# angelocatalani/neural-network-compression

Measured on AMD Instinct MI355X. Metric: weights/sec through prune+k-means (K=256), higher is better.
Workload: dtype f32

## Files before the change

### neural_network_compression_amd/csrc/nnc_hip.hip

```cpp
#include "nnc_common.hpp"
#include "nnc_km_shared.hpp"


extern "C" size_t nnc_kmeans_workspace_bytes(int32_t k)
{
    (void)k;
    return sizeof(KmWs) + 256;
}

extern "C" int32_t nnc_fix_shift(float absmax, int64_t n_total)
{
    int L = 1;
    while (((int64_t)1 << L) < n_total && L < 62) L++;
    if (!(absmax > 0.0f) || !std::isfinite(absmax)) return 0;
    int P = 0;
    (void)std::frexp((double)absmax, &P);
    return std::min(28, 62 - L) - P;
}

__device__ __forceinline__ int fix_f32(float v, int Sft)
{
    return (int)rintf(ldexpf(v, Sft));
}

// ... 3168 lines not shown
    unsigned char *b = reinterpret_cast<unsigned char *>(scratch_dev);
    float *cand_x = reinterpret_cast<float *>(b); b += reloc_align((size_t)cap * 4);
    float *cand_d = reinterpret_cast<float *>(b); b += reloc_align((size_t)cap * 4);
    KmWin *win = reinterpret_cast<KmWin *>(b); b += reloc_align(16 * (size_t)(p->k + 2));
    int *meta = reinterpret_cast<int *>(b); b += reloc_align(16);
    long long *keys = reinterpret_cast<long long *>(b); b += reloc_align(8 * (size_t)NNC_KMAX);
    unsigned *hist0 = reinterpret_cast<unsigned *>(b);
    int glog2, rlog2;
    km_defaults(p, &glog2, &rlog2);
    const size_t lds = km_lds_bytes(p->k, glog2, rlog2, false) + (NNC_KMAX + 2) * sizeof(int);
    if (lds > 128 * 1024) return fail(NNC_EINVAL, "relocation: search tables too large for the candidate kernel");
    if (!g_reloc_dist_attr[current_device()].load(std::memory_order_acquire)) {
        HIPCHK(hipFuncSetAttribute(reinterpret_cast<const void *>(&k_reloc_dist), hipFuncAttributeMaxDynamicSharedMemorySize, 128 * 1024));
        g_reloc_dist_attr[current_device()].store(1, std::memory_order_release);
    }
    NNC_LAUNCH_PROF(NNC_PROF_RELOC, k_reloc_head, dim3(KM_GMAX / KM_THREADS + 1), dim3(KM_THREADS), 0, S(stream), x_sorted, (long long)p->n, w, (long long)cap, win, meta,
                       hist0, (int)wmax);
    LAUNCHCHK("k_reloc_head");
    const int grid = (int)std::max<int64_t>(1, std::min<int64_t>(128, (2 * (int64_t)64 * (p->k + 1) + KM_THREADS - 1) / KM_THREADS));
    NNC_LAUNCH_PROF(NNC_PROF_RELOC, k_reloc_dist, dim3(grid), dim3(KM_THREADS), lds, S(stream), x_sorted, (const KmWin *)win, (const int *)meta, cand_x, cand_d, (long long)cap,
                       reinterpret_cast<const KmWs *>(w), hist0, 1);
    LAUNCHCHK("k_reloc_dist");
#ifndef KM_CHAIN_FIVE
    if (p->k > 256 && !km_fused(p) && p->prefix_dev) {
        unsigned char *hb = reinterpret_cast<unsigned char *>(host_mapped);
        NNC_LAUNCH_PROF(NNC_PROF_RELOC, k_reloc_select_finalize, dim3(1), dim3(KM_THREADS), 0, S(stream), w, (const float *)cand_x, (const float *)cand_d, (const KmWin *)win,
                        (const int *)meta, keys, (const unsigned *)hist0, reinterpret_cast<nnc_kmeans_status *>(hb),
                        reinterpret_cast<unsigned long long *>(hb ? hb + sizeof(nnc_kmeans_status) : nullptr), (unsigned long long)ticket, 1 | (p->k << 8));
        LAUNCHCHK("k_reloc_select_finalize");
        return NNC_OK;
    }
#endif
    NNC_LAUNCH_PROF(NNC_PROF_RELOC, k_reloc_select, dim3(1), dim3(KM_THREADS), 0, S(stream), w, (const float *)cand_x, (const float *)cand_d, (const KmWin *)win, (const int *)meta, 0, keys, 1, (const unsigned *)hist0, 1);
    LAUNCHCHK("k_reloc_select");
    return km_launch_finalize(w, p, FIN_FROM_PARTIALS, 2, stream, host_mapped, ticket);
}


int nnc_wait_ticket_(void *host_ticket, uint64_t ticket, void *stream)
{
    return km_wait_ticket(reinterpret_cast<volatile unsigned long long *>(host_ticket), (unsigned long long)ticket, S(stream));
}
int km_wait_ticket(volatile unsigned long long *word, unsigned long long ticket, hipStream_t stream)
{
    unsigned long long spins = 0;
    bool synced = false;
    auto t0 = std::chrono::steady_clock::now();
    while (__atomic_load_n(word, __ATOMIC_ACQUIRE) != ticket) {
        if ((++spins & 0x3FFF) == 0) {
            const double el = std::chrono::duration<double>(std::chrono::steady_clock::now() - t0).count();
            if (el > 0.02 && !synced) {
                hipError_t e = hipStreamSynchronize(stream);
                if (e != hipSuccess) return fail(NNC_EHIP, std::string("nnc_kmeans_fit: ") + hipGetErrorString(e));
                synced = true;
            } else if (el > 60.0) return fail(NNC_EHIP, "nnc_kmeans_fit: the status never arrived");
        }
    }
    return NNC_OK;
}

extern "C" int nnc_kmeans_fit(const float *x_iter, void *ws, const nnc_kmeans_params *pp, int32_t max_batch, int32_t sorted,
                              void *reloc_scratch_dev, size_t reloc_scratch_bytes, void *host_mapped, uint64_t *ticket_io,
                              nnc_kmeans_status *status_out, int32_t *n_windowed_out, void *stream)
{
    int rc = km_check(ws, pp, "nnc_kmeans_fit");
    if (rc) return rc;
    if (!host_mapped || !ticket_io || !status_out || (reinterpret_cast<uintptr_t>(host_mapped) & 7) != 0) return fail(NNC_EINVAL, "nnc_kmeans_fit: null / unaligned pointer");
    const nnc_kmeans_params p = *pp;
    if (p.n != p.n_total) return fail(NNC_EINVAL, "nnc_kmeans_fit: single GPU only (sharded fits: nnc_kmeans_iterate_sharded)");
    if (max_batch < 1) max_batch = 1;
    const bool lloyd = km_lloyd_ok(&p, x_iter);
    const bool one_launch = !lloyd && km_one_launch_fit(&p, x_iter);
    const size_t slot = sizeof(nnc_kmeans_status) + 8;
    unsigned char *hb = reinterpret_cast<unsigned char *>(host_mapped);
    const bool spec_ok = sorted && !one_launch && p.prefix_dev && reloc_scratch_dev && (reinterpret_cast<uintptr_t>(reloc_scratch_dev) & 255) == 0 &&
                         reloc_scratch_bytes >= nnc_kmeans_reloc_scratch_bytes(p.k, KM_SPEC_WMAX) && p.n >= 2 * KM_SPEC_WMAX;
    const bool mass_in_place = (p.flags & NNC_KM_MASS_IN_PLACE) && !lloyd && p.k > 64;
    bool spec = spec_ok && !mass_in_place;
    int batch = one_launch ? p.max_iter : (spec_ok ? 6 : 1);
    if (lloyd) batch = KM_LLOYD_ROUNDS;
    bool first_launch = true;
    int nwin = 0, nrel_seen = status_out->n_relocated, nunp_seen = status_out->n_unproven;
    int nip_seen = status_out->n_in_place;
    if (!spec_ok) { nrel_seen = 0; nunp_seen = 0; nip_seen = 0; }
    double s_prev = -1.0, s_last = -1.0;
    int i_prev = 0, i_last = 0;
    KmWs *w = reinterpret_cast<KmWs *>(ws);
    for (;;) {
        const uint64_t ticket = ++(*ticket_io);
        unsigned char *sl = hb + (ticket & 1) * slot;
        if (lloyd) {
            if ((rc = km_set_lds_attr())) return rc;
            for (int i = 0; i < batch; i++) {
                const bool last = i == batch - 1;
                if ((rc = km_launch_lloyd_round(x_iter, w, &p, first_launch ? p.max_iter : -1, stream, (last && !spec) ? sl : nullptr, ticket, spec ? 1 : 0))) return rc;
                first_launch = false;
                if (spec && (rc = km_launch_spec_reloc(x_iter, w, &p, reloc_scratch_dev, stream, last ? sl : nullptr, ticket))) return rc;
            }
        } else if (spec) {
            if ((rc = km_set_lds_attr())) return rc;
            for (int i = 0; i < batch; i++) {
                if ((rc = km_launch_accumulate(x_iter, w, &p, stream))) return rc;
                if ((rc = km_launch_finalize(w, &p, FIN_FROM_SHARDS, 0, stream, nullptr, 0, false, x_iter))) return rc;
                if ((rc = km_launch_spec_reloc(x_iter, w, &p, reloc_scratch_dev, stream, i == batch - 1 ? sl : nullptr, ticket))) return rc;
            }
        } else {
            const int lag = (!one_launch && batch >= 4) ? KM_FIT_LAG : 0;
            if ((rc = km_iterate_publish_(x_iter, ws, &p, batch, sl, ticket, stream, spec_ok, lag))) return rc;
        }
        if ((rc = km_wait_ticket(reinterpret_cast<volatile unsigned long long *>(sl + sizeof(nnc_kmeans_status)), ticket, S(stream)))) return rc;
        const nnc_kmeans_status st = *reinterpret_cast<const nnc_kmeans_status *>(sl);
        *status_out = st;
        const int dev_events = spec_ok ? st.n_relocated - nrel_seen : 0;
        const int chain_events = dev_events - (spec_ok ? st.n_in_place - nip_seen : 0);
        nrel_seen = st.n_relocated;
        nip_seen = st.n_in_place;
        nwin += dev_events;
        nwin += spec_ok ? st.n_unproven - nunp_seen : 0;
        nunp_seen = st.n_unproven;
        if (st.done) break;
        if (lloyd && !st.paused) continue;
        if (spec && !st.paused) {
            if (2 * chain_events >= batch) { batch = 4; s_prev = s_last = -1.0; continue; }
            spec = false;
            s_prev = s_last = -1.0;
        }
        if (st.paused) {
            const bool strict_check = st.iter >= 1 && st.same_counts;
            const int32_t window = (sorted && st.paused == 1 && !strict_check) ? nnc_kmeans_reloc_window(p.n, st.n_empty) : 0;
            if (window == 0 || !reloc_scratch_dev || reloc_scratch_bytes < nnc_kmeans_reloc_scratch_bytes(p.k, window)) break;
            if ((rc = nnc_kmeans_relocate_windowed(x_iter, ws, &p, st.n_empty, reloc_scratch_dev, reloc_scratch_bytes, stream))) return rc;
            nwin++;
            if (!lloyd) batch = one_launch ? p.max_iter : 1;
            s_prev = s_last = -1.0;
            continue;
        }
        if (one_launch) continue;
        s_prev = s_last; i_prev = i_last;
        s_last = (double)st.shift_tot; i_last = st.iter;
        batch = std::min(max_batch, batch * 2);
        if (s_prev > 0.0 && s_last > 0.0 && s_prev > s_last && p.tol > 0.0f) {
            const double rate = std::log(s_prev / s_last) / std::max(1, i_last - i_prev);
            const double left = s_last > (double)p.tol ? std::log(s_last / (double)p.tol) / rate : 0.0;
            batch = (int)std::max(1.0, std::min((double)max_batch, std::floor(left * 0.9)));
        }
    }
    if (n_windowed_out) *n_windowed_out = nwin;
    return NNC_OK;
}

extern "C" int nnc_kmeans_reloc_select_local(const float *x_sorted, void *ws, const nnc_kmeans_params *p, int32_t n_empty,
                                             void *scratch_dev, size_t scratch_bytes, int64_t *keys_out_dev, void *stream)
{
    int rc = km_check(ws, p, "nnc_kmeans_reloc_select_local");
    if (rc) return rc;
    const int32_t window = nnc_kmeans_reloc_window(p->n, n_empty);
    if (window == 0) return fail(NNC_EINVAL, "nnc_kmeans_reloc_select_local: not applicable (nnc_kmeans_reloc_window() == 0)");
    if (!x_sorted || !scratch_dev || !keys_out_dev || (reinterpret_cast<uintptr_t>(scratch_dev) & 255) != 0)
        return fail(NNC_EINVAL, "nnc_kmeans_reloc_select_local: null or unaligned (256 B) pointer");
    if (scratch_bytes < nnc_kmeans_reloc_scratch_bytes(p->k, window)) return fail(NNC_ENOSPACE, "nnc_kmeans_reloc_select_local: scratch too small");
    const int64_t cap = reloc_cap(p->k, window);
    unsigned char *b = reinterpret_cast<unsigned char *>(scratch_dev);
    float *cand_x = reinterpret_cast<float *>(b); b += reloc_align((size_t)cap * 4);
    float *cand_d = reinterpret_cast<float *>(b); b += reloc_align((size_t)cap * 4);
    void *win = b; b += reloc_align(16 * (size_t)(p->k + 2));
    int32_t *meta = reinterpret_cast<int32_t *>(b); b += reloc_align(16) + reloc_align(8 * (size_t)NNC_KMAX);
    unsigned *hist0 = reinterpret_cast<unsigned *>(b);
    if ((rc = km_reloc_windows_dist(x_sorted, ws, p, window, cand_x, cand_d, cap, win, meta, hist0, stream))) return rc;
    NNC_LAUNCH_PROF(NNC_PROF_RELOC, k_reloc_select, dim3(1), dim3(KM_THREADS), 0, S(stream), reinterpret_cast<KmWs *>(ws), cand_x, cand_d,
                       reinterpret_cast<const KmWin *>(win), reinterpret_cast<const int *>(meta), (int)n_empty,
                       reinterpret_cast<long long *>(keys_out_dev), 0, (const unsigned *)hist0, 0);
    LAUNCHCHK("k_reloc_select");
    return NNC_OK;
}

extern "C" int32_t *nnc_kmeans_reloc_flag(void *ws)
{
    if (!ws) return nullptr;
    return &reinterpret_cast<KmWs *>(ws)->reloc_fail;
}

__global__ __launch_bounds__(KM_THREADS) void k_relocate_if_proven(KmWs *__restrict__ ws, const long long *__restrict__ keys, int nkeys)
{
    __shared__ KmRelocLds lds;
    if (ws->reloc_fail) return;
    km_relocate_body(ws, keys, nkeys, &lds);
}

extern "C" int nnc_kmeans_relocate_if_proven(void *ws, const int64_t *keys_sorted_dev, int32_t nkeys, void *stream)
{
    if (!ws || !keys_sorted_dev || nkeys < 1) return fail(NNC_EINVAL, "nnc_kmeans_relocate_if_proven: bad argument");
    hipLaunchKernelGGL(k_relocate_if_proven, dim3(1), dim3(KM_THREADS), 0, S(stream), reinterpret_cast<KmWs *>(ws),
                       reinterpret_cast<const long long *>(keys_sorted_dev), nkeys);
    LAUNCHCHK("k_relocate_if_proven");
    return NNC_OK;
}

template <typename LT>
__global__ __launch_bounds__(256) void k_labels_equal(const LT *__restrict__ a, const LT *__restrict__ b, int64_t n, int *flag)
{
    const int64_t tid = (int64_t)blockIdx.x * blockDim.x + threadIdx.x;
    const int64_t nthreads = (int64_t)gridDim.x * blockDim.x;
    int diff = 0;
    for (int64_t i = tid; i < n; i += nthreads) diff |= (a[i] != b[i]);
    if (__any(diff) && (threadIdx.x & 63) == 0) *flag = 0;
}
__global__ void k_set_i32(int *p, int v) { *p = v; }
__global__ void k_set_done_if(KmWs *ws, const int *flag, int code) { if (*flag) ws->st.done = code; }

extern "C" int nnc_labels_equal(const void *a, const void *b, int64_t n, int label_bytes, int32_t *flag_dev, void *stream)
{
    if (!flag_dev || n < 0 || (n > 0 && (!a || !b))) return fail(NNC_EINVAL, "nnc_labels_equal: bad argument");
    hipLaunchKernelGGL(k_set_i32, dim3(1), dim3(1), 0, S(stream), flag_dev, 1);
    LAUNCHCHK("k_set_i32");
    if (n == 0) return NNC_OK;
    const int64_t bytes = n * label_bytes;
    if (((reinterpret_cast<uintptr_t>(a) | reinterpret_cast<uintptr_t>(b)) & 7) == 0 && (bytes & 7) == 0) {
        int grid = stream_grid(bytes / 8, 256 * 4, 8);
        hipLaunchKernelGGL((k_labels_equal<unsigned long long>), dim3(grid), dim3(256), 0, S(stream), reinterpret_cast<const unsigned long long *>(a), reinterpret_cast<const unsigned long long *>(b), bytes / 8, flag_dev);
    } else if (label_bytes == 1) {
        int grid = stream_grid(n, 256 * 4, 8);
        hipLaunchKernelGGL((k_labels_equal<uint8_t>), dim3(grid), dim3(256), 0, S(stream), reinterpret_cast<const uint8_t *>(a), reinterpret_cast<const uint8_t *>(b), n, flag_dev);
    } else {
        int grid = stream_grid(n, 256 * 4, 8);
        hipLaunchKernelGGL((k_labels_equal<uint16_t>), dim3(grid), dim3(256), 0, S(stream), reinterpret_cast<const uint16_t *>(a), reinterpret_cast<const uint16_t *>(b), n, flag_dev);
    }
    LAUNCHCHK("k_labels_equal");
// ... 64 lines not shown
```

### neural_network_compression_amd/csrc/nnc_layer.hip

```cpp
#include <hip/hip_runtime.h>

#include <algorithm>
#include <cmath>
#include <cstdint>
#include <cstring>
#include <string>
#include <vector>

#include "nnc.h"

int nnc_set_error_(int code, const char *msg);
int nnc_publish_bytes_(const void *src_dev, void *dst_host_mapped, int nbytes, void *host_ticket, uint64_t ticket, void *stream);
int nnc_wait_ticket_(void *host_ticket, uint64_t ticket, void *stream);
int nnc_sort_pruned_bounded_flagged_(const float *x, int64_t n, int64_t n_neg, int64_t n_zero, float vmin, float vmax, float thr,
                                     float *sorted_out, void *ws, size_t ws_bytes, int32_t *flag_dev, void *stream);

extern "C" int nnc_host_linspace_f32(float start, float stop, int32_t num, float *out)
{
    if (num < 0 || (num > 0 && !out)) return nnc_set_error_(NNC_EINVAL, "nnc_host_linspace_f32: bad argument");
    if (num == 0) return NNC_OK;
    const int div = num - 1;
    const volatile float delta = stop - start;
    if (div > 0) {
        const volatile float step = delta / (float)div;
        for (int i = 0; i < num; i++) {
            volatile float y = (float)i;
            if (step == 0.0f) { y = y / (float)div; y = y * delta; }
            else y = y * step;
            y = y + start;
            out[i] = y;
        }
        out[num - 1] = stop;
    } else {
        volatile float y = 0.0f;
        y = y * delta;
        y = y + start;
        out[0] = y;
    }
    return NNC_OK;
}

static void linspace_f64(double start, double stop, int num, double *out)
{
    const int div = num - 1;
    const volatile double delta = stop - start;
    if (div > 0) {
        const volatile double step = delta / (double)div;
        for (int i = 0; i < num; i++) {
            volatile double y = (double)i;
            if (step == 0.0) { y = y / (double)div; y = y * delta; }
            else y = y * step;
            y = y + start;
            out[i] = y;
        }
        out[num - 1] = stop;
    } else if (num == 1) {
        volatile double y = 0.0;
        y = y * delta;
        out[0] = y + start;
    }
}

extern "C" int nnc_host_cdf(const float *steps32, const int64_t *counts31, float *xnew300, double *cdf300)
{
    if (!steps32 || !counts31 || !xnew300 || !cdf300) return nnc_set_error_(NNC_EINVAL, "nnc_host_cdf: null pointer");
    const float *x = steps32;
    int64_t tot = 0;
    for (int i = 0; i < 31; i++) tot += counts31[i];
    double cdf[31];
    volatile double acc = 0.0;
    for (int i = 0; i < 31; i++) {
        const volatile double t = (double)counts31[i] / (double)tot;
        acc = (i == 0) ? (double)t : acc + t;
        cdf[i] = acc;
    }
    const double last = cdf[30];
    for (int i = 0; i < 31; i++) { const volatile double q = cdf[i] / last; cdf[i] = q; }
    float xmin = x[0], xmax = x[0];
    for (int i = 1; i < 31; i++) { xmin = std::min(xmin, x[i]); xmax = std::max(xmax, x[i]); }
    int rc = nnc_host_linspace_f32(xmin, xmax, 300, xnew300);
    if (rc) return rc;
    for (int j = 0; j < 300; j++) {
        const float v = xnew300[j];
        int idx = (int)(std::lower_bound(x, x + 31, v) - x);
        idx = std::min(std::max(idx, 1), 30);
        const int lo = idx - 1, hi = idx;
        const volatile float dx = x[hi] - x[lo];
        const volatile double dy = cdf[hi] - cdf[lo];
        const volatile double slope = dy / (double)dx;
        const volatile float xr = v - x[lo];
        const volatile double prod = slope * (double)xr;
        cdf300[j] = prod + cdf[lo];
    }
    return NNC_OK;
}

extern "C" int nnc_host_density_init(const float *xnew300, const double *cdf300, int32_t bits, float *space_out)
{
    if (!xnew300 || !cdf300 || !space_out || bits < 0 || bits > 10) return nnc_set_error_(NNC_EINVAL, "nnc_host_density_init: bad argument");
    const int k = (1 << bits) + 1;
    std::vector<double> tmp((size_t)k);
    linspace_f64(0.0, 1.0, k, tmp.data());
    for (int t = 0; t < k; t++) {
        int best = 0;
        double bd = std::fabs(cdf300[0] - tmp[t]);
        for (int j = 1; j < 300; j++) {
            const double d = std::fabs(cdf300[j] - tmp[t]);
            if (d < bd) { bd = d; best = j; }
        }
        space_out[t] = xnew300[best];
    }
    return NNC_OK;
}

static size_t al(size_t b) { return (b + 255) & ~(size_t)255; }

struct SideStream { int dev = -1; hipStream_t stream = nullptr; hipEvent_t fork = nullptr, join = nullptr; };
static int side_stream(SideStream **out)
{
    static thread_local SideStream side;
    int dev = 0;
    if (hipGetDevice(&dev) != hipSuccess) return nnc_set_error_(NNC_EHIP, "hipGetDevice failed");
    if (side.dev != dev) {
        if (side.stream) { (void)hipStreamDestroy(side.stream); (void)hipEventDestroy(side.fork); (void)hipEventDestroy(side.join); side = SideStream(); }
        if (hipStreamCreateWithFlags(&side.stream, hipStreamNonBlocking) != hipSuccess || hipEventCreateWithFlags(&side.fork, hipEventDisableTiming) != hipSuccess ||
            hipEventCreateWithFlags(&side.join, hipEventDisableTiming) != hipSuccess)
            return nnc_set_error_(NNC_EHIP, "could not create the second stream");
        side.dev = dev;
    }
    *out = &side;
    return NNC_OK;
}

struct LayerLayout {
    size_t prune_ws, stats_out, stats_ws, sorted, sort_ws, km_ws, prefix, reloc, back, small_out, total;
    size_t prune_ws_bytes, stats_ws_bytes, sort_ws_bytes, km_ws_bytes, prefix_bytes, reloc_bytes;
};

static LayerLayout layer_layout(int64_t n, int32_t k)
{
    LayerLayout L;
    size_t o = 0;
    auto take = [&](size_t bytes) { const size_t at = o; o += al(bytes); return at; };
    L.prune_ws_bytes = nnc_prune_stats_workspace_bytes(n);
    L.stats_ws_bytes = std::max(nnc_layer_stats_workspace_bytes(n), nnc_minmax_workspace_bytes(n));
    L.sort_ws_bytes = std::max(std::max(nnc_sort_workspace_bytes(n), nnc_sort_pruned_workspace_bytes(n, 0, (n + 3) / 4)),
                               nnc_sort_pruned_bounded_workspace_bytes(n - (n + 3) / 4));
    L.km_ws_bytes = nnc_kmeans_workspace_bytes(k);
    L.prefix_bytes = nnc_kmeans_prefix_bytes(n);
    L.reloc_bytes = n >= 512 ? nnc_kmeans_reloc_scratch_bytes(k, 256) : 0;
    L.prune_ws = take(std::max<size_t>(L.prune_ws_bytes, 16));
    L.stats_out = take(512);
    L.stats_ws = take(std::max<size_t>(L.stats_ws_bytes, 16));
    L.sorted = take((size_t)n * 4 + 16);
    L.sort_ws = take(std::max<size_t>(L.sort_ws_bytes, 16));
    L.km_ws = take(L.km_ws_bytes);
    L.prefix = take(std::max<size_t>(L.prefix_bytes, 16));
    L.reloc = take(std::max<size_t>(L.reloc_bytes, 16));
    L.back = take((size_t)k * 12);
    L.small_out = take(64 + 256);
    L.total = o + 256;
    return L;
}

extern "C" size_t nnc_compress_layer_workspace_bytes(int64_t n, int32_t k)
{
    if (n < 1 || k < 1 || k > NNC_KMAX - 8) return 0;
    return layer_layout(n, k).total;
}

extern "C" size_t nnc_compress_layer_host_bytes(void) { return 24576; }

#define LCHK(call) do { int rc_ = (call); if (rc_) return rc_; } while (0)
#define LHIP(call) do { hipError_t e_ = (call); if (e_ != hipSuccess) return nnc_set_error_(NNC_EHIP, hipGetErrorString(e_)); } while (0)

extern "C" int nnc_compress_layer_f32(float *x, int64_t n, const nnc_layer_params *lp, uint8_t *mask_out, void *labels_out,
                                      float *values_out, void *ws_dev, size_t ws_bytes, void *host_pinned, size_t host_bytes,
                                      uint64_t *ticket_io, nnc_layer_result *res, void *stream)
{
    if (!x || n < 1 || !lp || !labels_out || !ws_dev || !host_pinned || !ticket_io || !res)
        return nnc_set_error_(NNC_EINVAL, "nnc_compress_layer_f32: null pointer or empty tensor");
    if (lp->bits < 1 || lp->bits > 10 || (lp->mode != NNC_INIT_LINEAR && lp->mode != NNC_INIT_DENSITY))
        return nnc_set_error_(NNC_EINVAL, "nnc_compress_layer_f32: bits in 1..10, mode linear or density");
    if (lp->prune && !mask_out) return nnc_set_error_(NNC_EINVAL, "nnc_compress_layer_f32: pruning needs mask_out");
    const int32_t k = (1 << lp->bits) + (lp->mode == NNC_INIT_DENSITY ? 1 : 0);
    if (n < (int64_t)(1 << lp->bits) + 1) return nnc_set_error_(NNC_EINVAL, "nnc_compress_layer_f32: not enough weights for this many centroids");
    if (host_bytes < nnc_compress_layer_host_bytes() || (reinterpret_cast<uintptr_t>(host_pinned) & 7) != 0)
        return nnc_set_error_(NNC_EINVAL, "nnc_compress_layer_f32: host block too small or unaligned");
    const LayerLayout L = layer_layout(n, k);
    if (ws_bytes < L.total) return nnc_set_error_(NNC_ENOSPACE, "nnc_compress_layer_f32: workspace too small");
    hipStream_t s = reinterpret_cast<hipStream_t>(stream);
    unsigned char *wb = reinterpret_cast<unsigned char *>((reinterpret_cast<uintptr_t>(ws_dev) + 255) & ~(uintptr_t)255);
    unsigned char *hb = reinterpret_cast<unsigned char *>(host_pinned);
    const float *h_f = reinterpret_cast<const float *>(hb + 512);
    const int64_t *h_signs = reinterpret_cast<const int64_t *>(hb + 512 + 32);
    const float *h_prune = reinterpret_cast<const float *>(hb + 512 + 48);
    const int64_t *h_nz = reinterpret_cast<const int64_t *>(hb + 512 + 56);
    int64_t *h_ranks = reinterpret_cast<int64_t *>(hb + 576);
    void *h_ticket = hb + 504;
    auto read_back = [&](const void *src, void *dst, int nbytes) -> int {
        const uint64_t t = ++(*ticket_io);
        int rc = nnc_publish_bytes_(src, dst, nbytes, h_ticket, t, stream);
        if (rc) return rc;
        return nnc_wait_ticket_(h_ticket, t, stream);
    };
    std::memset(res, 0, sizeof(*res));
    res->k = k;
    res->label_bytes = k <= 256 ? 1 : 2;

    float *out6 = reinterpret_cast<float *>(wb + L.stats_out);
    int64_t *signs = reinterpret_cast<int64_t *>(wb + L.stats_out + 32);
    float *pstats = reinterpret_cast<float *>(wb + L.stats_out + 48);
    int64_t *nzeroed = reinterpret_cast<int64_t *>(wb + L.stats_out + 56);
    if (lp->prune)
        LCHK(nnc_prune_stats_f32(x, n, lp->q, lp->std_smooth ? 1 : 0, mask_out, pstats, nzeroed, out6 + 2, signs, wb + L.prune_ws, L.prune_ws_bytes, stream));
    else
        LCHK(nnc_minmax_signs_f32(x, n, out6 + 2, signs, wb + L.stats_ws, L.stats_ws_bytes, stream));
    const bool short_tensor = n <= NNC_REF_NMAX && k <= NNC_REF_KMAX;
    if ((short_tensor && lp->mode != NNC_INIT_LINEAR) || (!short_tensor && n < 512)) {
        if (lp->prune) {
            LCHK(read_back(out6, hb + 512, 64));
            res->sigma = h_prune[0]; res->threshold = h_prune[1]; res->n_zeroed = h_nz[0];
        }
        res->status = NNC_LAYER_HOST;
        return NNC_OK;
    }
    float space[NNC_KMAX];
    unsigned char *back = wb + L.back;
    int64_t *counts_d = reinterpret_cast<int64_t *>(back);
    float *centers_d = reinterpret_cast<float *>(back + (size_t)k * 8);
    int64_t *h_counts = reinterpret_cast<int64_t *>(hb + 1024);
    float *h_centers = reinterpret_cast<float *>(hb + 1024 + (size_t)k * 8);
    float *h_steps = reinterpret_cast<float *>(hb + 896), *h_space = reinterpret_cast<float *>(hb + 16384);

    if (short_tensor) {
        LCHK(read_back(out6, hb + 512, 64));
        LCHK(nnc_host_linspace_f32(h_f[2], h_f[3], k, space));
        std::memcpy(h_space, space, (size_t)k * 4);
        void *result_d = wb + L.small_out;
        LCHK(nnc_kmeans_fit_reference_f32(x, (int32_t)n, h_space, k, 300, 1e-4f, reinterpret_cast<uint8_t *>(labels_out), lp->want_values ? values_out : nullptr,
                                          centers_d, counts_d, result_d, stream));
        const int back_bytes = (int)al((size_t)k * 12) + 32;
        LCHK(read_back(back, hb + 1024, back_bytes));
        const int32_t *h_res = reinterpret_cast<const int32_t *>(hb + 1024 + al((size_t)k * 12));
        {
            const float *h_resf = reinterpret_cast<const float *>(h_res);
            if (!std::isfinite(h_resf[6]) || !std::isfinite(h_resf[7])) {
                if (lp->prune) { res->sigma = h_prune[0]; res->threshold = h_prune[1]; res->n_zeroed = h_nz[0]; }
                res->status = NNC_LAYER_HOST;
                return NNC_OK;
            }
        }
        res->n_iter = h_res[0]; res->stop = h_res[1]; res->n_relocations = h_res[2]; res->reloc_ties = h_res[3]; res->reloc_multi = h_res[4];
        res->arith = NNC_ARITH_REFERENCE;
    } else {
        const int64_t nch = (n + 8191) / 8192;
        float *c1 = reinterpret_cast<float *>(wb + L.stats_ws), *c2 = c1 + nch;
        LCHK(read_back(out6, hb + 512, 64));
        const float xmin = h_f[2], xmax = h_f[3], min_nz = h_f[4], max_nz = h_f[5];
        const int64_t n_neg = h_signs[0], n_zero = h_signs[1];
        SideStream *side = nullptr;
        LCHK(side_stream(&side));
        LHIP(hipEventRecord(side->fork, s));
        LHIP(hipStreamWaitEvent(side->stream, side->fork, 0));
        struct SideJoin {
            SideStream *side; hipStream_t s; bool joined = false;
            ~SideJoin() { if (!joined) { (void)hipEventRecord(side->join, side->stream); (void)hipStreamWaitEvent(s, side->join, 0); (void)hipStreamSynchronize(s); } }
        } side_join{side, s};
        LCHK(nnc_chunk_sums_f32(x, n, 0, nullptr, c1, side->stream));
        LCHK(nnc_fold_f32(c1, nch, n, NNC_FOLD_MEAN, nullptr, out6, side->stream));
        LCHK(nnc_chunk_sums_f32(x, n, 1, out6, c2, side->stream));
        LCHK(nnc_fold_f32(c2, nch, n, NNC_FOLD_MEAN, nullptr, out6 + 1, side->stream));
        void *h_ticket_side = hb + 864;
        const float *h_mv = reinterpret_cast<const float *>(hb + 872);
        const uint64_t t_mv = ++(*ticket_io);
        LCHK(nnc_publish_bytes_(out6, hb + 872, 8, h_ticket_side, t_mv, side->stream));
        LHIP(hipEventRecord(side->join, side->stream));
        float *xs = reinterpret_cast<float *>(wb + L.sorted);
        int32_t *oob_d = reinterpret_cast<int32_t *>(wb + L.stats_out + 336);
        const int32_t *h_oob = reinterpret_cast<const int32_t *>(hb + 512 + 336);
        bool bounded = false;
        if (4 * n_zero >= n && lp->prune && nnc_sort_pruned_bounded_bits(xmin, xmax, h_prune[1], n_neg, n - n_neg - n_zero) > 0) {
            LCHK(nnc_sort_pruned_bounded_flagged_(x, n, n_neg, n_zero, xmin, xmax, h_prune[1], xs, wb + L.sort_ws, L.sort_ws_bytes, oob_d, stream));
            bounded = true;
        } else if (4 * n_zero >= n) LCHK(nnc_sort_pruned_f32(x, n, n_neg, n_zero, xs, wb + L.sort_ws, L.sort_ws_bytes, stream));
        else LCHK(nnc_sort_f32(x, n, xs, wb + L.sort_ws, L.sort_ws_bytes, stream));
        const bool with_prefix = (reinterpret_cast<uintptr_t>(xs) & 15) == 0;
        int64_t *ranks_d = reinterpret_cast<int64_t *>(wb + L.stats_out + 64);
        h_ranks = reinterpret_cast<int64_t *>(hb + 512 + 64);
        float steps[32];
        if (lp->mode == NNC_INIT_DENSITY) {
            if (!std::isfinite(min_nz)) {
                LHIP(hipStreamWaitEvent(s, side->join, 0));
                LHIP(hipStreamSynchronize(s));
                side_join.joined = true;
                if (lp->prune) { res->sigma = h_prune[0]; res->threshold = h_prune[1]; res->n_zeroed = h_nz[0]; }
                res->status = NNC_LAYER_HOST;
                return NNC_OK;
            }
            LCHK(nnc_host_linspace_f32(min_nz, max_nz, 32, steps));
            std::memcpy(h_steps, steps, 128);
            LCHK(nnc_rank_sorted_f32(xs, n, h_steps, 32, ranks_d, stream));
        }
        const uint64_t t_rk = ++(*ticket_io);
        LCHK(nnc_publish_bytes_(out6 + 2, hb + 512 + 8, 56 + 33 * 8 + 16, h_ticket, t_rk, stream));
        LCHK(nnc_wait_ticket_(h_ticket_side, t_mv, side->stream));
        LHIP(hipStreamWaitEvent(s, side->join, 0));
        side_join.joined = true;
        const float mean = h_mv[0], var = h_mv[1];
        if (!std::isfinite(mean) || !std::isfinite(var) || !std::isfinite(xmin) || !std::isfinite(xmax)) {
            LCHK(nnc_wait_ticket_(h_ticket, t_rk, stream));
            if (lp->prune) { res->sigma = h_prune[0]; res->threshold = h_prune[1]; res->n_zeroed = h_nz[0]; }
            res->status = NNC_LAYER_HOST;
            return NNC_OK;
        }
        nnc_kmeans_params p;
        std::memset(&p, 0, sizeof(p));
        const volatile float tol = var * 1e-4f;
        const volatile float lo = xmin - mean, hi = xmax - mean;
        p.n = n; p.n_total = n; p.k = k; p.max_iter = 300;
        p.fix_shift = nnc_fix_shift(std::max(std::fabs((float)lo), std::fabs((float)hi)), n);
        p.grid_log2 = 0; p.replicas_log2 = -1; p.flags = lp->km_flags & (NNC_KM_TWO_LAUNCH | NNC_KM_LOOP);
        p.x_mean = mean; p.tol = tol; p.lo = lo; p.hi = hi;
        if (with_prefix) {
            LCHK(nnc_kmeans_prefix_build(xs, &p, reinterpret_cast<int64_t *>(wb + L.prefix), stream));
            p.prefix_dev = reinterpret_cast<int64_t *>(wb + L.prefix);
        }
        LCHK(nnc_wait_ticket_(h_ticket, t_rk, stream));
        if (bounded && *h_oob) {
            if (lp->prune) { res->sigma = h_prune[0]; res->threshold = h_prune[1]; res->n_zeroed = h_nz[0]; }
            res->status = NNC_LAYER_HOST;
            return NNC_OK;
        }
        if (lp->mode == NNC_INIT_LINEAR) {
            LCHK(nnc_host_linspace_f32(xmin, xmax, k, space));
        } else {
            int64_t counts31[31];
            for (int b = 0; b < 31; b++) counts31[b] = h_ranks[b + 1] - h_ranks[b];
            for (int b = 0; b < 31; b++)
                if (steps[b] <= 0.0f && 0.0f < steps[b + 1]) { counts31[b] -= n_zero; break; }
            float xnew[300];
            double cdf[300];
            LCHK(nnc_host_cdf(steps, counts31, xnew, cdf));
            LCHK(nnc_host_density_init(xnew, cdf, lp->bits, space));
        }
        std::memcpy(h_space, space, (size_t)k * 4);
        LCHK(nnc_kmeans_init(wb + L.km_ws, L.km_ws_bytes, &p, h_space, stream));
        nnc_kmeans_status st;
        std::memset(&st, 0, sizeof(st));
        int32_t nwin = 0;
        LCHK(nnc_kmeans_fit(xs, wb + L.km_ws, &p, 16, 1, L.reloc_bytes ? wb + L.reloc : nullptr, L.reloc_bytes, hb, ticket_io, &st, &nwin, stream));
        if (!st.done) {
            if (lp->prune) { res->sigma = h_prune[0]; res->threshold = h_prune[1]; res->n_zeroed = h_nz[0]; }
            res->status = NNC_LAYER_HOST;
            return NNC_OK;
        }
        LCHK(nnc_kmeans_get_centers(wb + L.km_ws, 0, 0, centers_d, stream));
        LCHK(nnc_kmeans_assign(x, wb + L.km_ws, &p, 0, labels_out, res->label_bytes, lp->want_values ? values_out : nullptr, nullptr, nullptr, stream));
        LCHK(nnc_kmeans_label_counts(xs, wb + L.km_ws, &p, 0, counts_d, stream));
        LCHK(read_back(back, hb + 1024, (int)al((size_t)k * 12)));
        res->n_iter = st.iter; res->stop = st.done; res->n_relocations = nwin - st.n_reloc_null; res->n_reloc_windowed = nwin - st.n_reloc_null;
        res->reloc_ties = st.reloc_ties; res->reloc_multi = st.reloc_multi;
        res->arith = NNC_ARITH_FIXED;
    }
    if (lp->prune) { res->sigma = h_prune[0]; res->threshold = h_prune[1]; res->n_zeroed = h_nz[0]; }
    std::memcpy(res->counts, h_counts, (size_t)k * 8);
    std::memcpy(res->centers, h_centers, (size_t)k * 4);
    int64_t hist[72];
    LCHK(nnc_huffman_lengths(res->counts, k, res->code_lengths, hist, &res->total_bits));
    res->status = NNC_LAYER_DONE;
    return NNC_OK;
}
```

### neural_network_compression_amd/csrc/nnc_sort.hip

```cpp
#include <hip/hip_runtime.h>
#include <cmath>
#include <cstdlib>
#include <cstring>

#include <algorithm>
#include <string>

#include "nnc.h"

extern "C" const char *nnc_last_error(void);
int nnc_set_error_(int code, const char *msg);

#ifndef OS_THREADS
#define OS_THREADS 1024
#endif
#define OS_WAVES (OS_THREADS / 64)
#ifndef OS_ITEMS
#define OS_ITEMS 16
#endif
#ifndef OS_BLOCKS_PER_CU
#define OS_BLOCKS_PER_CU 1
#endif
#ifndef OS_RANK_LDS
#define OS_RANK_LDS 1
// ... 302 lines not shown
                keys_s[(unsigned)tpre[d] + (unsigned)wcnt[wv][d] + (unsigned)rnk[i]] = key[i];
            }
        }
        OS_STAMP(3);
        if (DST == 1 && n_zero > 0) {
            const long long per = ((n_zero + ntiles - 1) / ntiles + 3) & ~3ll;
            const long long z0 = tile * per, z1 = (z0 + per < n_zero) ? z0 + per : n_zero;
            float *zp = out_f + n_neg;
            if ((reinterpret_cast<uintptr_t>(zp) & 15) == 0) {
                for (long long i = z0 + 4ll * t; i + 3 < z1; i += 4ll * OS_THREADS) *reinterpret_cast<float4 *>(zp + i) = make_float4(0.f, 0.f, 0.f, 0.f);
                if (t == 0) for (long long i = z0 + ((z1 - z0) & ~3ll); i < z1; i++) zp[i] = 0.0f;
            } else {
                for (long long i = z0 + t; i < z1; i += OS_THREADS) zp[i] = 0.0f;
            }
        }
#pragma unroll
        for (int r = 0; r < DPT; r++) {
            const int d = t * DPT + r;
            if (d >= R) continue;
            unsigned excl = 0;
            if (tile > 0 && !(abl & 1)) {
                long long i = tile - 1;
                int polls = 0;
                bool done = false;
                while (!done) {
                    unsigned long long w[OS_LOOK];
#pragma unroll
                    for (int j = 0; j < OS_LOOK; j++) w[j] = (i - j >= 0) ? os_peek(&status[(size_t)(i - j) * R + d]) : 0ull;
                    int used = 0;
#pragma unroll
                    for (int j = 0; j < OS_LOOK; j++) {
                        if (!done && used == j) {
                            const unsigned tg = (unsigned)(w[j] >> 32);
                            if (tg == tagP) { excl += (unsigned)w[j]; done = true; }
                            else if (tg == tagA) { excl += (unsigned)w[j]; used = j + 1; }
                        }
                    }
                    if (!done) {
                        i -= used;
                        if (used == 0) {
                            if (++polls > OS_SPIN_LIMIT) { gave_up = true; done = true; }
                            __builtin_amdgcn_s_sleep(1);
                        } else polls = 0;
                    }
                }
                os_publish(&status[(size_t)tile * R + d], tagP, excl + tc[r]);
            }
            gpos[d] = gdig[d] + excl - (unsigned)tpre[d];
        }
        OS_STAMP(4);
        __syncthreads();
        OS_STAMP(5);
        for (int j = t; j < cnt_tile; j += OS_THREADS) {
            const unsigned kv = keys_s[j];
            const unsigned d = (kv >> shift) & MASK;
            const unsigned r = gpos[d] + (unsigned)j;
            if ((long long)r < n && !(abl & 4)) {
                if (DST == 0) out_k[r] = kv;
                else out_f[(long long)r + ((long long)r >= n_neg ? n_zero : 0)] = os_value(km, kv);
            }
        }
        OS_STAMP(6);
        __syncthreads();
        OS_STAMP(7);
    }
    if (gave_up) atomicOr(ctrl + 1, 2ull);
    if (nrb > 0) {
        for (int i = t; i <= (int)nmask; i += OS_THREADS) {
            const unsigned v = nhist[i];
            if (v) atomicAdd(&ghist_next[i], v);
        }
    }
}

static unsigned host_ord(float v)
{
    unsigned b;
    std::memcpy(&b, &v, 4);
    return (b & 0x80000000u) ? ~b : (b | 0x80000000u);
}

static size_t al256(size_t b) { return (b + 255) & ~(size_t)255; }

static int os_cus()
{
    static int cus[64] = {0};
    int dev = 0;
    if (hipGetDevice(&dev) != hipSuccess || dev < 0 || dev >= 64) return 256;
    if (!cus[dev]) {
        int v = 0;
        if (hipDeviceGetAttribute(&v, hipDeviceAttributeMultiprocessorCount, dev) != hipSuccess || v <= 0) v = 256;
        cus[dev] = v;
    }
    return cus[dev];
}

static OsPlan os_plan(int bits)
{
    OsPlan pl;
    std::memset(&pl, 0, sizeof(pl));
    int rb;
    if (bits <= 8) { pl.passes = 1; rb = 8; }
    else if (bits <= 16) { pl.passes = 2; rb = 8; }
    else if (bits <= 18) { pl.passes = 2; rb = 9; }
    else if (bits <= 24) { pl.passes = 3; rb = 8; }
    else if (bits <= 27) { pl.passes = 3; rb = 9; }
    else { pl.passes = 4; rb = 8; }
    for (int p = 0; p < pl.passes; p++) { pl.shift[p] = p * rb; pl.rb[p] = rb; }
    return pl;
}

static size_t os_status_bytes(int64_t n_keys)
{
    const int64_t ntiles = (n_keys + OS_TILE - 1) / OS_TILE;
    return al256((size_t)std::max<int64_t>(ntiles, 1) * OS_MAXR * 8);
}
static size_t os_ws_bytes(int64_t n_keys)
{
    return 2 * al256((size_t)n_keys * 4 + 16) + al256(OS_CTRL_WORDS * 8) + al256((size_t)(OS_MAXPASS + 1) * OS_MAXR * 4) + os_status_bytes(n_keys) + 256;
}
static unsigned char *os_ws_base(void *ws) { return reinterpret_cast<unsigned char *>((reinterpret_cast<uintptr_t>(ws) + 255) & ~(uintptr_t)255); }

static int os_sort(const float *x, int64_t n, bool skip_zeros, int64_t n_neg, int64_t n_zero, const OsMap &km, int bits, float *sorted_out, void *ws,
                   size_t ws_bytes, int32_t *flag_dev, const char *who, void *stream)
{
    const int64_t n_keys = skip_zeros ? n - n_zero : n;
    if (!ws || ws_bytes < os_ws_bytes(n_keys)) return nnc_set_error_(NNC_ENOSPACE, (std::string(who) + ": workspace too small").c_str());
    hipStream_t s = reinterpret_cast<hipStream_t>(stream);
    unsigned char *b = os_ws_base(ws);
    unsigned *ka = reinterpret_cast<unsigned *>(b); b += al256((size_t)n_keys * 4 + 16);
    unsigned *kb = reinterpret_cast<unsigned *>(b); b += al256((size_t)n_keys * 4 + 16);
    unsigned long long *ctrl = reinterpret_cast<unsigned long long *>(b); b += al256(OS_CTRL_WORDS * 8);
    unsigned *ghist = reinterpret_cast<unsigned *>(b); b += al256((size_t)(OS_MAXPASS + 1) * OS_MAXR * 4);
    unsigned long long *status = reinterpret_cast<unsigned long long *>(b);
    hipError_t e;
    const size_t zero_bytes = al256(OS_CTRL_WORDS * 8) + al256((size_t)(OS_MAXPASS + 1) * OS_MAXR * 4) + os_status_bytes(n_keys);
    if ((e = hipMemsetAsync(ctrl, 0, zero_bytes, s)) != hipSuccess) return nnc_set_error_(NNC_EHIP, hipGetErrorString(e));
    if (skip_zeros && n_zero > 0 && n_keys == 0 && (e = hipMemsetAsync(sorted_out + n_neg, 0, (size_t)n_zero * 4, s)) != hipSuccess) return nnc_set_error_(NNC_EHIP, hipGetErrorString(e));
    const OsPlan pl = os_plan(bits);
    int abl = 0;
#ifdef NNC_DIAG
    { const char *ev = getenv("NNC_OS_ABLATE"); abl = ev ? atoi(ev) : 0; }
#endif
    if (n_keys > 0) {
        const long long ptiles = (n + OSP_TILE - 1) / OSP_TILE;
        const int pgrid = (int)std::min<long long>(std::max<long long>(ptiles, 1), 2LL * os_cus());
        if (skip_zeros) hipLaunchKernelGGL((k_os_prep<true>), dim3(pgrid), dim3(OSP_THREADS), 0, s, x, (long long)n, ka, ctrl, (long long)n_keys, km, pl.rb[0], ghist);
        else hipLaunchKernelGGL((k_os_prep<false>), dim3(pgrid), dim3(OSP_THREADS), 0, s, x, (long long)n, (unsigned *)nullptr, ctrl, (long long)n_keys, km, pl.rb[0], ghist);
        if ((e = hipGetLastError()) != hipSuccess) return nnc_set_error_(NNC_EHIP, hipGetErrorString(e));
        const long long ntiles = (n_keys + OS_TILE - 1) / OS_TILE;
        const int grid = (int)std::min<long long>(ntiles, (long long)OS_BLOCKS_PER_CU * os_cus());
        const void *src = skip_zeros ? (const void *)ka : (const void *)x;
        unsigned *dst = skip_zeros ? kb : ka;
        for (int p = 0; p < pl.passes; p++) {
            const bool first_f = (p == 0 && !skip_zeros), last = (p == pl.passes - 1);
            void *o = last ? (void *)sorted_out : (void *)dst;
#define OS_LAUNCH(SRC, DST) do { \
                if (pl.rb[p] == 9) hipLaunchKernelGGL((k_os_pass<9, SRC, DST>), dim3(grid), dim3(OS_THREADS), 0, s, src, o, (long long)n_keys, pl.shift[p], p, last ? 0 : pl.rb[p + 1], \
                                                      ghist + (size_t)p * OS_MAXR, ghist + (size_t)(p + 1) * OS_MAXR, status, ctrl, km, (long long)(skip_zeros ? n_neg : n_keys), (long long)(skip_zeros ? n_zero : 0), abl); \
                else hipLaunchKernelGGL((k_os_pass<8, SRC, DST>), dim3(grid), dim3(OS_THREADS), 0, s, src, o, (long long)n_keys, pl.shift[p], p, last ? 0 : pl.rb[p + 1], \
                                        ghist + (size_t)p * OS_MAXR, ghist + (size_t)(p + 1) * OS_MAXR, status, ctrl, km, (long long)(skip_zeros ? n_neg : n_keys), (long long)(skip_zeros ? n_zero : 0), abl); \
            } while (0)
            if (first_f && last) OS_LAUNCH(1, 1);
            else if (first_f) OS_LAUNCH(1, 0);
            else if (last) OS_LAUNCH(0, 1);
            else OS_LAUNCH(0, 0);
#undef OS_LAUNCH
            if ((e = hipGetLastError()) != hipSuccess) return nnc_set_error_(NNC_EHIP, hipGetErrorString(e));
            src = dst;
            dst = (dst == ka) ? kb : ka;
        }
    }
    if (flag_dev && (e = hipMemcpyAsync(flag_dev, reinterpret_cast<unsigned char *>(ctrl) + 8, 4, hipMemcpyDeviceToDevice, s)) != hipSuccess)
        return nnc_set_error_(NNC_EHIP, hipGetErrorString(e));
    return NNC_OK;
}

static OsMap os_identity()
{
    OsMap m;
    std::memset(&m, 0, sizeof(m));
    return m;
}

extern "C" size_t nnc_sort_workspace_bytes(int64_t n) { return n <= 0 ? 0 : os_ws_bytes(n); }

extern "C" int nnc_sort_f32(const float *x, int64_t n, float *sorted_out, void *ws, size_t ws_bytes, void *stream)
{
    if (n < 0 || n >= ((int64_t)1 << 31) || (n > 0 && (!x || !sorted_out))) return nnc_set_error_(NNC_EINVAL, "nnc_sort_f32: bad argument");
    if (n == 0) return NNC_OK;
    return os_sort(x, n, false, 0, 0, os_identity(), 32, sorted_out, ws, ws_bytes, nullptr, "nnc_sort_f32", stream);
}

extern "C" size_t nnc_sort_pruned_workspace_bytes(int64_t n, int64_t n_neg, int64_t n_zero)
{
    if (n <= 0 || n_neg < 0 || n_zero < 0 || n_neg + n_zero > n) return 0;
    return os_ws_bytes(n - n_zero);
}

extern "C" int nnc_sort_pruned_f32(const float *x, int64_t n, int64_t n_neg, int64_t n_zero, float *sorted_out, void *ws,
                                   size_t ws_bytes, void *stream)
{
    if (n < 0 || n_neg < 0 || n_zero < 0 || n_neg + n_zero > n || n >= ((int64_t)1 << 31) || (n > 0 && (!x || !sorted_out)))
        return nnc_set_error_(NNC_EINVAL, "nnc_sort_pruned_f32: bad argument");
    if (n == 0) return NNC_OK;
    return os_sort(x, n, true, n_neg, n_zero, os_identity(), 32, sorted_out, ws, ws_bytes, nullptr, "nnc_sort_pruned_f32", stream);
}

static int rs_bounds(float vmin, float vmax, float thr, int64_t n_neg, int64_t n_pos, OsMap *bd)
{
    if (!(thr > 0.0f) || !std::isfinite(thr) || !std::isfinite(vmin) || !std::isfinite(vmax)) return 0;
    OsMap b;
    std::memset(&b, 0, sizeof(b));
    b.bounded = 1;
    unsigned long long total = 0;
    if (n_neg > 0) {
        if (!(vmin <= -thr)) return 0;
        b.lo_neg = host_ord(vmin); b.hi_neg = host_ord(-thr);
        b.span_neg = b.hi_neg - b.lo_neg + 1u;
        total += b.span_neg;
    }
    if (n_pos > 0) {
        if (!(vmax >= thr)) return 0;
        b.lo_pos = host_ord(thr); b.hi_pos = host_ord(vmax);
        total += (unsigned long long)(b.hi_pos - b.lo_pos) + 1ull;
    }
    if (total == 0 || total > (1ull << 27)) return 0;
    int bits = 1;
    while ((1ull << bits) < total) bits++;
    *bd = b;
    return bits;
}

extern "C" int32_t nnc_sort_pruned_bounded_bits(float vmin, float vmax, float thr, int64_t n_neg, int64_t n_pos)
{
    OsMap b;
    return rs_bounds(vmin, vmax, thr, n_neg, n_pos, &b);
}

extern "C" size_t nnc_sort_pruned_bounded_workspace_bytes(int64_t n_nz)
{
    if (n_nz < 0) return 0;
    return os_ws_bytes(n_nz);
}

int nnc_sort_pruned_bounded_flagged_(const float *x, int64_t n, int64_t n_neg, int64_t n_zero, float vmin, float vmax, float thr,
                                     float *sorted_out, void *ws, size_t ws_bytes, int32_t *flag_dev, void *stream);
extern "C" int nnc_sort_pruned_bounded_f32(const float *x, int64_t n, int64_t n_neg, int64_t n_zero, float vmin, float vmax, float thr,
                                           float *sorted_out, void *ws, size_t ws_bytes, void *stream)
{
    return nnc_sort_pruned_bounded_flagged_(x, n, n_neg, n_zero, vmin, vmax, thr, sorted_out, ws, ws_bytes, nullptr, stream);
}

extern "C" const int32_t *nnc_sort_pruned_bounded_flag(void *ws, int64_t n_nonzero)
{
    if (!ws || n_nonzero < 0) return nullptr;
    unsigned char *b = os_ws_base(ws) + 2 * al256((size_t)n_nonzero * 4 + 16);
// ... 18 lines not shown
```

Baseline: 10.05 billion.

## Overlap host readbacks, move prefix build to side stream, replace memset/memcpy with kernels

Several independent latency cuts in the per-layer prune+k-means path. A blocking readback of the min/max stats becomes an async ticket publish, and the prefix build moves to the side stream so it overlaps the main stream. The label-count readback is published before the assign kernel rather than after it. The density-init nearest-CDF search switches from a linear scan to binary search. The sort's memset and device-to-device memcpy become small custom kernels. The k-means fit loop also changes its batch and lag heuristics, including where the speculative-relocation status is published, which alters the iteration schedule and could change convergence behaviour.

```diff
diff --git a/neural_network_compression_amd/csrc/nnc_hip.hip b/neural_network_compression_amd/csrc/nnc_hip.hip
--- a/neural_network_compression_amd/csrc/nnc_hip.hip
+++ b/neural_network_compression_amd/csrc/nnc_hip.hip
@@ -3274,6 +3274,7 @@
     bool first_launch = true;
     int nwin = 0, nrel_seen = status_out->n_relocated, nunp_seen = status_out->n_unproven;
     int nip_seen = status_out->n_in_place;
+    int spec_seen = 0, spec_unseen = 0;
     if (!spec_ok) { nrel_seen = 0; nunp_seen = 0; nip_seen = 0; }
     double s_prev = -1.0, s_last = -1.0;
     int i_prev = 0, i_last = 0;
@@ -3291,13 +3292,16 @@
             }
         } else if (spec) {
             if ((rc = km_set_lds_attr())) return rc;
+            const int carry = batch >= 2 ? batch - 2 : batch - 1;
+            spec_seen = spec_unseen + carry + 1;
+            spec_unseen = batch - 1 - carry;
             for (int i = 0; i < batch; i++) {
                 if ((rc = km_launch_accumulate(x_iter, w, &p, stream))) return rc;
                 if ((rc = km_launch_finalize(w, &p, FIN_FROM_SHARDS, 0, stream, nullptr, 0, false, x_iter))) return rc;
-                if ((rc = km_launch_spec_reloc(x_iter, w, &p, reloc_scratch_dev, stream, i == batch - 1 ? sl : nullptr, ticket))) return rc;
+                if ((rc = km_launch_spec_reloc(x_iter, w, &p, reloc_scratch_dev, stream, i == carry ? sl : nullptr, ticket))) return rc;
             }
         } else {
-            const int lag = (!one_launch && batch >= 4) ? KM_FIT_LAG : 0;
+            const int lag = one_launch ? 0 : std::min(KM_FIT_LAG, batch - 1);
             if ((rc = km_iterate_publish_(x_iter, ws, &p, batch, sl, ticket, stream, spec_ok, lag))) return rc;
         }
         if ((rc = km_wait_ticket(reinterpret_cast<volatile unsigned long long *>(sl + sizeof(nnc_kmeans_status)), ticket, S(stream)))) return rc;
@@ -3313,7 +3317,7 @@
         if (st.done) break;
         if (lloyd && !st.paused) continue;
         if (spec && !st.paused) {
-            if (2 * chain_events >= batch) { batch = 4; s_prev = s_last = -1.0; continue; }
+            if (2 * chain_events > spec_seen) { batch = 4; s_prev = s_last = -1.0; continue; }
             spec = false;
             s_prev = s_last = -1.0;
         }
@@ -3334,7 +3338,7 @@
         if (s_prev > 0.0 && s_last > 0.0 && s_prev > s_last && p.tol > 0.0f) {
             const double rate = std::log(s_prev / s_last) / std::max(1, i_last - i_prev);
             const double left = s_last > (double)p.tol ? std::log(s_last / (double)p.tol) / rate : 0.0;
-            batch = (int)std::max(1.0, std::min((double)max_batch, std::floor(left * 0.9)));
+            batch = (int)std::max((double)std::min(max_batch, KM_FIT_LAG + 1), std::min((double)max_batch, std::floor(left * 0.9)));
         }
     }
     if (n_windowed_out) *n_windowed_out = nwin;
diff --git a/neural_network_compression_amd/csrc/nnc_layer.hip b/neural_network_compression_amd/csrc/nnc_layer.hip
--- a/neural_network_compression_amd/csrc/nnc_layer.hip
+++ b/neural_network_compression_amd/csrc/nnc_layer.hip
@@ -14,7 +14,6 @@
 int nnc_wait_ticket_(void *host_ticket, uint64_t ticket, void *stream);
 int nnc_sort_pruned_bounded_flagged_(const float *x, int64_t n, int64_t n_neg, int64_t n_zero, float vmin, float vmax, float thr,
                                      float *sorted_out, void *ws, size_t ws_bytes, int32_t *flag_dev, void *stream);
-
 extern "C" int nnc_host_linspace_f32(float start, float stop, int32_t num, float *out)
 {
     if (num < 0 || (num > 0 && !out)) return nnc_set_error_(NNC_EINVAL, "nnc_host_linspace_f32: bad argument");
@@ -101,6 +100,21 @@
     const int k = (1 << bits) + 1;
     std::vector<double> tmp((size_t)k);
     linspace_f64(0.0, 1.0, k, tmp.data());
+    bool rising = true;
+    for (int j = 1; j < 300; j++) rising = rising && cdf300[j - 1] <= cdf300[j];
+    for (int t = 0; rising && t < k; t++) {
+        const int hi = (int)(std::lower_bound(cdf300, cdf300 + 300, tmp[t]) - cdf300);
+        int best = hi;
+        if (hi > 0) {
+            const double dl = std::fabs(cdf300[hi - 1] - tmp[t]);
+            if (hi == 300 || dl <= std::fabs(cdf300[hi] - tmp[t])) {
+                best = hi - 1;
+                while (best > 0 && std::fabs(cdf300[best - 1] - tmp[t]) == dl) best--;
+            }
+        }
+        space_out[t] = xnew300[best];
+    }
+    if (rising) return NNC_OK;
     for (int t = 0; t < k; t++) {
         int best = 0;
         double bd = std::fabs(cdf300[0] - tmp[t]);
@@ -115,16 +129,16 @@
 
 static size_t al(size_t b) { return (b + 255) & ~(size_t)255; }
 
-struct SideStream { int dev = -1; hipStream_t stream = nullptr; hipEvent_t fork = nullptr, join = nullptr; };
+struct SideStream { int dev = -1; hipStream_t stream = nullptr; hipEvent_t fork = nullptr, sorted = nullptr, join = nullptr; };
 static int side_stream(SideStream **out)
 {
     static thread_local SideStream side;
     int dev = 0;
     if (hipGetDevice(&dev) != hipSuccess) return nnc_set_error_(NNC_EHIP, "hipGetDevice failed");
     if (side.dev != dev) {
-        if (side.stream) { (void)hipStreamDestroy(side.stream); (void)hipEventDestroy(side.fork); (void)hipEventDestroy(side.join); side = SideStream(); }
+        if (side.stream) { (void)hipStreamDestroy(side.stream); (void)hipEventDestroy(side.fork); (void)hipEventDestroy(side.sorted); (void)hipEventDestroy(side.join); side = SideStream(); }
         if (hipStreamCreateWithFlags(&side.stream, hipStreamNonBlocking) != hipSuccess || hipEventCreateWithFlags(&side.fork, hipEventDisableTiming) != hipSuccess ||
-            hipEventCreateWithFlags(&side.join, hipEventDisableTiming) != hipSuccess)
+            hipEventCreateWithFlags(&side.sorted, hipEventDisableTiming) != hipSuccess || hipEventCreateWithFlags(&side.join, hipEventDisableTiming) != hipSuccess)
             return nnc_set_error_(NNC_EHIP, "could not create the second stream");
         side.dev = dev;
     }
@@ -256,12 +270,11 @@
     } else {
         const int64_t nch = (n + 8191) / 8192;
         float *c1 = reinterpret_cast<float *>(wb + L.stats_ws), *c2 = c1 + nch;
-        LCHK(read_back(out6, hb + 512, 64));
-        const float xmin = h_f[2], xmax = h_f[3], min_nz = h_f[4], max_nz = h_f[5];
-        const int64_t n_neg = h_signs[0], n_zero = h_signs[1];
         SideStream *side = nullptr;
         LCHK(side_stream(&side));
         LHIP(hipEventRecord(side->fork, s));
+        const uint64_t t_mm = ++(*ticket_io);
+        LCHK(nnc_publish_bytes_(out6 + 2, hb + 512 + 8, 56, h_ticket, t_mm, stream));
         LHIP(hipStreamWaitEvent(side->stream, side->fork, 0));
         struct SideJoin {
             SideStream *side; hipStream_t s; bool joined = false;
@@ -275,7 +288,9 @@
         const float *h_mv = reinterpret_cast<const float *>(hb + 872);
         const uint64_t t_mv = ++(*ticket_io);
         LCHK(nnc_publish_bytes_(out6, hb + 872, 8, h_ticket_side, t_mv, side->stream));
-        LHIP(hipEventRecord(side->join, side->stream));
+        LCHK(nnc_wait_ticket_(h_ticket, t_mm, stream));
+        const float xmin = h_f[2], xmax = h_f[3], min_nz = h_f[4], max_nz = h_f[5];
+        const int64_t n_neg = h_signs[0], n_zero = h_signs[1];
         float *xs = reinterpret_cast<float *>(wb + L.sorted);
         int32_t *oob_d = reinterpret_cast<int32_t *>(wb + L.stats_out + 336);
         const int32_t *h_oob = reinterpret_cast<const int32_t *>(hb + 512 + 336);
@@ -285,15 +300,13 @@
             bounded = true;
         } else if (4 * n_zero >= n) LCHK(nnc_sort_pruned_f32(x, n, n_neg, n_zero, xs, wb + L.sort_ws, L.sort_ws_bytes, stream));
         else LCHK(nnc_sort_f32(x, n, xs, wb + L.sort_ws, L.sort_ws_bytes, stream));
+        LHIP(hipEventRecord(side->sorted, s));
         const bool with_prefix = (reinterpret_cast<uintptr_t>(xs) & 15) == 0;
         int64_t *ranks_d = reinterpret_cast<int64_t *>(wb + L.stats_out + 64);
         h_ranks = reinterpret_cast<int64_t *>(hb + 512 + 64);
         float steps[32];
         if (lp->mode == NNC_INIT_DENSITY) {
             if (!std::isfinite(min_nz)) {
-                LHIP(hipStreamWaitEvent(s, side->join, 0));
-                LHIP(hipStreamSynchronize(s));
-                side_join.joined = true;
                 if (lp->prune) { res->sigma = h_prune[0]; res->threshold = h_prune[1]; res->n_zeroed = h_nz[0]; }
                 res->status = NNC_LAYER_HOST;
                 return NNC_OK;
@@ -305,8 +318,6 @@
         const uint64_t t_rk = ++(*ticket_io);
         LCHK(nnc_publish_bytes_(out6 + 2, hb + 512 + 8, 56 + 33 * 8 + 16, h_ticket, t_rk, stream));
         LCHK(nnc_wait_ticket_(h_ticket_side, t_mv, side->stream));
-        LHIP(hipStreamWaitEvent(s, side->join, 0));
-        side_join.joined = true;
         const float mean = h_mv[0], var = h_mv[1];
         if (!std::isfinite(mean) || !std::isfinite(var) || !std::isfinite(xmin) || !std::isfinite(xmax)) {
             LCHK(nnc_wait_ticket_(h_ticket, t_rk, stream));
@@ -323,9 +334,11 @@
         p.grid_log2 = 0; p.replicas_log2 = -1; p.flags = lp->km_flags & (NNC_KM_TWO_LAUNCH | NNC_KM_LOOP);
         p.x_mean = mean; p.tol = tol; p.lo = lo; p.hi = hi;
         if (with_prefix) {
-            LCHK(nnc_kmeans_prefix_build(xs, &p, reinterpret_cast<int64_t *>(wb + L.prefix), stream));
+            LHIP(hipStreamWaitEvent(side->stream, side->sorted, 0));
+            LCHK(nnc_kmeans_prefix_build(xs, &p, reinterpret_cast<int64_t *>(wb + L.prefix), side->stream));
             p.prefix_dev = reinterpret_cast<int64_t *>(wb + L.prefix);
         }
+        LHIP(hipEventRecord(side->join, side->stream));
         LCHK(nnc_wait_ticket_(h_ticket, t_rk, stream));
         if (bounded && *h_oob) {
             if (lp->prune) { res->sigma = h_prune[0]; res->threshold = h_prune[1]; res->n_zeroed = h_nz[0]; }
@@ -346,6 +359,8 @@
         }
         std::memcpy(h_space, space, (size_t)k * 4);
         LCHK(nnc_kmeans_init(wb + L.km_ws, L.km_ws_bytes, &p, h_space, stream));
+        LHIP(hipStreamWaitEvent(s, side->join, 0));
+        side_join.joined = true;
         nnc_kmeans_status st;
         std::memset(&st, 0, sizeof(st));
         int32_t nwin = 0;
@@ -356,9 +371,11 @@
             return NNC_OK;
         }
         LCHK(nnc_kmeans_get_centers(wb + L.km_ws, 0, 0, centers_d, stream));
+        LCHK(nnc_kmeans_label_counts(xs, wb + L.km_ws, &p, 0, counts_d, stream));
+        const uint64_t t_back = ++(*ticket_io);
+        LCHK(nnc_publish_bytes_(back, hb + 1024, (int)al((size_t)k * 12), h_ticket, t_back, stream));
         LCHK(nnc_kmeans_assign(x, wb + L.km_ws, &p, 0, labels_out, res->label_bytes, lp->want_values ? values_out : nullptr, nullptr, nullptr, stream));
-        LCHK(nnc_kmeans_label_counts(xs, wb + L.km_ws, &p, 0, counts_d, stream));
-        LCHK(read_back(back, hb + 1024, (int)al((size_t)k * 12)));
+        LCHK(nnc_wait_ticket_(h_ticket, t_back, stream));
         res->n_iter = st.iter; res->stop = st.done; res->n_relocations = nwin - st.n_reloc_null; res->n_reloc_windowed = nwin - st.n_reloc_null;
         res->reloc_ties = st.reloc_ties; res->reloc_multi = st.reloc_multi;
         res->arith = NNC_ARITH_FIXED;
diff --git a/neural_network_compression_amd/csrc/nnc_sort.hip b/neural_network_compression_amd/csrc/nnc_sort.hip
--- a/neural_network_compression_amd/csrc/nnc_sort.hip
+++ b/neural_network_compression_amd/csrc/nnc_sort.hip
@@ -408,6 +408,13 @@
 
 static size_t al256(size_t b) { return (b + 255) & ~(size_t)255; }
 
+__global__ __launch_bounds__(256) void k_os_clear(uint4 *__restrict__ p, long long n16)
+{
+    const long long stride = (long long)gridDim.x * 256;
+    for (long long i = (long long)blockIdx.x * 256 + threadIdx.x; i < n16; i += stride) p[i] = make_uint4(0u, 0u, 0u, 0u);
+}
+__global__ void k_os_verdict(const unsigned long long *__restrict__ ctrl, int32_t *__restrict__ flag) { *flag = reinterpret_cast<const int32_t *>(ctrl)[2]; }
+
 static int os_cus()
 {
     static int cus[64] = {0};
@@ -461,7 +468,9 @@
     unsigned long long *status = reinterpret_cast<unsigned long long *>(b);
     hipError_t e;
     const size_t zero_bytes = al256(OS_CTRL_WORDS * 8) + al256((size_t)(OS_MAXPASS + 1) * OS_MAXR * 4) + os_status_bytes(n_keys);
-    if ((e = hipMemsetAsync(ctrl, 0, zero_bytes, s)) != hipSuccess) return nnc_set_error_(NNC_EHIP, hipGetErrorString(e));
+    const long long n16 = (long long)(zero_bytes / 16);
+    hipLaunchKernelGGL(k_os_clear, dim3((unsigned)std::min<long long>((n16 + 255) / 256, 1024)), dim3(256), 0, s, reinterpret_cast<uint4 *>(ctrl), n16);
+    if ((e = hipGetLastError()) != hipSuccess) return nnc_set_error_(NNC_EHIP, hipGetErrorString(e));
     if (skip_zeros && n_zero > 0 && n_keys == 0 && (e = hipMemsetAsync(sorted_out + n_neg, 0, (size_t)n_zero * 4, s)) != hipSuccess) return nnc_set_error_(NNC_EHIP, hipGetErrorString(e));
     const OsPlan pl = os_plan(bits);
     int abl = 0;
@@ -497,8 +506,10 @@
             dst = (dst == ka) ? kb : ka;
         }
     }
-    if (flag_dev && (e = hipMemcpyAsync(flag_dev, reinterpret_cast<unsigned char *>(ctrl) + 8, 4, hipMemcpyDeviceToDevice, s)) != hipSuccess)
-        return nnc_set_error_(NNC_EHIP, hipGetErrorString(e));
+    if (flag_dev) {
+        hipLaunchKernelGGL(k_os_verdict, dim3(1), dim3(1), 0, s, (const unsigned long long *)ctrl, flag_dev);
+        if ((e = hipGetLastError()) != hipSuccess) return nnc_set_error_(NNC_EHIP, hipGetErrorString(e));
+    }
     return NNC_OK;
 }
 
```

Measured after the change: 10.48 billion (median of 6 runs). 4.3% higher.
